# alexncoleman/WeaklySupervisedDL

Hardware: AMD Instinct MI355X
Metric: SegmentationModel train img/s at B=16 256x256 (higher is better)
Workload: dtype f32

## Files before the change

### include/wsdl_hip.h

```cpp
#ifndef WSDL_HIP_H
#define WSDL_HIP_H

#include <stddef.h>
#include <stdint.h>

#ifdef __cplusplus
extern "C" {
#endif

typedef void* wsdl_stream_t;

enum {
    WSDL_OK = 0,
    WSDL_EINVAL = -1,
    WSDL_EHIP = -2,
    WSDL_EWORKSPACE = -3
};

const char* wsdl_last_error(void);
int wsdl_launch_trace(int on);
const char* wsdl_last_launches(void);
int wsdl_version(void);
const char* wsdl_target_arch(void);

int wsdl_set_option(const char* name, int value);

enum { WSDL_PROF_IGEMM_128x128_A = 0,
       WSDL_PROF_IGEMM_128x128_U = 1,
       WSDL_PROF_IGEMM_128x64_A = 2, WSDL_PROF_IGEMM_128x64_U = 3,
       WSDL_PROF_IGEMM_64x256_A = 4, WSDL_PROF_IGEMM_64x256_U = 5,
       WSDL_PROF_IGEMM_64x128_A = 6, WSDL_PROF_IGEMM_64x128_U = 7,
       WSDL_PROF_WGRAD_128x128 = 8,
       WSDL_PROF_WGRAD_64x128 = 9,
       WSDL_PROF_WGRAD_FAST_128x128 = 10,
       WSDL_PROF_PAIRWISE = 11, WSDL_PROF_LAYERCAM = 12,
       WSDL_PROF_SPLIT_128x128 = 13,
       WSDL_PROF_SPLIT_128x64 = 14, WSDL_PROF_SPLIT_64x256 = 15, WSDL_PROF_SPLIT_64x128 = 16,
       WSDL_PROF_WGRAD_SPLIT32 = 17,
       WSDL_PROF_SPLIT_256x128 = 18,
       WSDL_PROF_STEM = 19,
       WSDL_PROF_WGRAD_SPLIT16D = 20,
       WSDL_PROF_SPLIT_GROUP = 21,
       WSDL_PROF_SPLIT_MULTI = 22,
       WSDL_PROF_NCLASSES = 23 };
const char* wsdl_prof_class_name(int cls);
int wsdl_prof_enable(int on);
int wsdl_prof_collect(int cls, long long* launches, double* total_ms, double* total_work,
                      double* total_work_executed ,
                      double* total_bytes );
int wsdl_prof_reset(void);

int wsdl_range_enable(int on);
int wsdl_range_push(const char* name);
int wsdl_range_pop(void);


size_t wsdl_conv2d_weight_layout_bytes(int Cout, int Cin, int kh, int kw, int dgrad, int* is_plain);
int wsdl_conv2d_prep_weights(const float* w, void* wt_fwd, void* wt_dgrad,
                             int Cout, int Cin, int kh, int kw,
                             const float* w_amax ,
                             wsdl_stream_t stream);

int wsdl_conv2d_fwd(const float* x, const void* wt_fwd, float* y,
                    int B, int Cin, int H, int W, int Cout, int kh, int kw,
                    int stride, int pad, int dil,
                    const float* scale, const float* shift, const float* residual, int relu,
                    long long x_bs, long long y_bs, long long res_bs,
                    const float* x_amax ,
                    float* y_amax ,
                    void* ws, size_t ws_bytes, wsdl_stream_t stream);
typedef struct wsdl_prep_desc {
    const float* w;
    void* wt_fwd;
    void* wt_dgrad;
    const float* w_amax;
    int Cout, Cin, taps, grid_x;
    int block_begin, reserved;
} wsdl_prep_desc;
int wsdl_conv2d_prep_weights_multi(const wsdl_prep_desc* desc, int n, int total_blocks, wsdl_stream_t stream);

size_t wsdl_conv2d_igemm_workspace(int B, int Cin, int H, int W, int Cout, int kh, int kw,
                                   int stride, int pad, int dil, int dgrad);

int wsdl_conv2d_dgrad(const float* dy, const void* wt_dgrad, float* dx,
                      int B, int Cin, int H, int W, int Cout, int kh, int kw,
                      int stride, int pad, int dil, int accumulate, const uint8_t* acc_mask,
                      long long dy_bs, const float* dy_amax, void* ws, size_t ws_bytes, wsdl_stream_t stream);
int wsdl_conv2d_fwd_group_ok(int n, int B, int Cin, int H, int W, int Cout);
size_t wsdl_conv2d_fwd_group_workspace(int n, const int* k, const int* dil, int B, int Cin, int H, int W, int Cout);
int wsdl_conv2d_fwd_group(int n, const float* x, const void* const* wt_fwd, float* const* y, const int* k, const int* dil,
                          int B, int Cin, int H, int W, int Cout, long long x_bs, const long long* y_bs,
                          const float* x_amax, void* ws, size_t ws_bytes, wsdl_stream_t stream);
int wsdl_conv2d_dgrad_multi_ok(int n, int B, int Cin, int H, int W, int Cout);
int wsdl_conv2d_dgrad_multi(int n, const float* const* dy, const void* const* wt_dgrad, const float* const* dy_amax,
                            const int* k, const int* dil, const long long* dy_bs, float* dx, int B, int Cin, int H, int W,
                            int Cout, int accumulate, wsdl_stream_t stream);

size_t wsdl_conv2d_wgrad_workspace(int B, int Cin, int H, int W, int Cout, int kh, int kw,
                                   int stride, int pad, int dil);
int wsdl_conv2d_wgrad(const float* x, const float* dy, float* dw,
                      int B, int Cin, int H, int W, int Cout, int kh, int kw,
                      int stride, int pad, int dil, int accumulate,
                      long long x_bs, long long dy_bs, const float* x_amax, const float* dy_amax,
                      void* ws, size_t ws_bytes, wsdl_stream_t stream);
size_t wsdl_conv2d_wgrad_presplit_bytes(int B, int Cin, int H, int W, int Cout, int kh, int kw, int stride, int pad, int dil);
int wsdl_conv2d_wgrad_ex(const float* x, const float* dy, float* dw, int B, int Cin, int H, int W,
                         int Cout, int kh, int kw, int stride, int pad, int dil, int accumulate,
                         long long x_bs, long long dy_bs, const float* x_amax, const float* dy_amax,
                         const float* x_chan_amax, const float* dy_chan_amax, const void* dy_presplit, void* ws,
                         size_t ws_bytes, wsdl_stream_t stream);

int wsdl_amax(const float* x, int B, long long per_image, long long x_bs, float* out, int zero_first,
              wsdl_stream_t stream);
int wsdl_multi_amax(const float* const* ptrs, const long long* counts, int n, float* out, wsdl_stream_t stream);

int wsdl_bias_grad(const float* dy, float* dbias, int B, int C, int HW, long long dy_bs,
                   int accumulate, wsdl_stream_t stream);

size_t wsdl_bn_workspace(int C);
int wsdl_bn_train_fwd(const float* x, const float* gamma, const float* beta, float* y,
                      float* save_mean, float* save_invstd, float* running_mean, float* running_var,
                      float momentum, float eps, int B, int C, int HW,
                      const float* residual, int relu, long long y_bs,
                      float* y_amax ,
                      uint8_t* relu_mask ,
                      void* ws, size_t ws_bytes,
                      float* chan_amax ,
// ... 365 lines not shown
```

### weaklysuperviseddl_amd/csrc/common.hip

```cpp
#include "common.h"

#include <dlfcn.h>

#include <algorithm>
#include <mutex>
#include <vector>

namespace wsdl {

static thread_local char g_err[512] = "";
Opt g_range_sentinel{0};

void set_error(const char* fmt, ...) {
    va_list ap;
    va_start(ap, fmt);
    vsnprintf(g_err, sizeof(g_err), fmt, ap);
    va_end(ap);
}

std::atomic<int> g_trace_launches{0};
static thread_local char g_trace[2048] = "";
static thread_local size_t g_trace_len = 0;
void trace_launch(const char* fmt, ...) {
    if (g_trace_len + 4 >= sizeof(g_trace)) return;
// ... 17 lines not shown
bool prof_enabled() { return g_prof_on; }

static bool g_ranges_on = false;
static int (*g_roctx_push)(const char*) = nullptr;
static int (*g_roctx_pop)() = nullptr;
static bool load_roctx() {
    if (g_roctx_push && g_roctx_pop) return true;
    for (const char* name : {"librocprofiler-sdk-roctx.so", "librocprofiler-sdk-roctx.so.1", "libroctx64.so", "libroctx64.so.4"}) {
        if (void* h = dlopen(name, RTLD_NOW | RTLD_GLOBAL)) {
            g_roctx_push = reinterpret_cast<int (*)(const char*)>(dlsym(h, "roctxRangePushA"));
            g_roctx_pop = reinterpret_cast<int (*)()>(dlsym(h, "roctxRangePop"));
            if (g_roctx_push && g_roctx_pop) return true;
        }
    }
    return false;
}

ProfScope::ProfScope(int c, hipStream_t st, double work, double work_executed, double bytes)
    : cls(c), s(st), slot(nullptr) {
    if (g_ranges_on) g_roctx_push(wsdl_prof_class_name(c));
    if (!g_prof_on) return;
    std::lock_guard<std::mutex> lk(g_prof_mu);
    ProfRec r;
    r.work = work;
    r.executed = work_executed >= 0.0 ? work_executed : work;
    r.bytes = bytes;
    if (!g_free_events.empty()) {
        r.start = g_free_events.back().first;
        r.stop = g_free_events.back().second;
        g_free_events.pop_back();
    } else {
        if (hipEventCreate(&r.start) != hipSuccess) return;
        if (hipEventCreate(&r.stop) != hipSuccess) return;
    }
    (void)hipEventRecord(r.start, s);
    g_prof[cls].push_back(r);
    slot = reinterpret_cast<void*>(g_prof[cls].size());
}

ProfScope::~ProfScope() {
    if (g_ranges_on) g_roctx_pop();
    if (!slot) return;
    std::lock_guard<std::mutex> lk(g_prof_mu);
    size_t idx = reinterpret_cast<size_t>(slot) - 1;
    if (idx < g_prof[cls].size()) (void)hipEventRecord(g_prof[cls][idx].stop, s);
}

}

extern "C" {

int wsdl_launch_trace(int on) {
    wsdl::g_trace_launches.store(on ? 1 : 0);
    wsdl::g_trace[0] = 0;
    wsdl::g_trace_len = 0;
    return WSDL_OK;
}

const char* wsdl_last_launches(void) {
    static thread_local char out[sizeof(wsdl::g_trace)];
    memcpy(out, wsdl::g_trace, sizeof(out));
    wsdl::g_trace[0] = 0;
    wsdl::g_trace_len = 0;
    return out;
}

const char* wsdl_last_error(void) { return wsdl::g_err; }
int wsdl_version(void) { return 201; }
const char* wsdl_target_arch(void) { return "gfx950"; }

const char* wsdl_prof_class_name(int cls) {
    static const char* names[WSDL_PROF_NCLASSES] = {
        "conv_igemm_fast_kernel<128, 128, 2, 16>", "conv_igemm_kernel<128, 128, 2, false>",
        "conv_igemm_fast_kernel<128, 64, 2, 32>", "conv_igemm_kernel<128, 64, 2, false>",
        "conv_igemm_fast_kernel<64, 256, 1, 16>", "conv_igemm_kernel<64, 256, 1, false>",
        "conv_igemm_fast_kernel<64, 128, 1, 32>", "conv_igemm_kernel<64, 128, 1, false>",
        "conv_wgrad_kernel<128, 128, 2>", "conv_wgrad_kernel<64, 128, 1>", "conv_wgrad_fast_kernel<128, 128, 2, 16>",
        "pairwise_kernel", "layercam_partial_kernel",
        "conv_igemm_split_kernel<128, 128, 2, 16, 256, AR>", "conv_igemm_split_kernel<128, 64, 2, 32, 256, AR>",
        "conv_igemm_split_kernel<64, 256, 1, 16, 256, AR>", "conv_igemm_split_kernel<64, 128, 1, 32, 256, AR>",
        "conv_wgrad_split16_kernel<128, 128, false>", "conv_igemm_split_kernel<256, 128, 4, BK, 512, AR, false, false>",
        "stem_conv7x7s2_kernel", "conv_wgrad_split16d_kernel<MODE, DYRAW>",
        "conv_igemm_split_group_kernel<256, 128, 4, 16, 512, AR, false>",
        "conv_igemm_split_kernel<256, 128, 4, 16, 512, AR, false, true>"};
    return cls >= 0 && cls < WSDL_PROF_NCLASSES ? names[cls] : "?";
}

int wsdl_range_enable(int on) {
    if (on && !wsdl::load_roctx()) {
        wsdl::set_error("range_enable: librocprofiler-sdk-roctx.so / libroctx64.so could not be loaded");
        return WSDL_EINVAL;
    }
    wsdl::g_ranges_on = on != 0;
    return WSDL_OK;
}
int wsdl_range_push(const char* name) {
    if (wsdl::g_ranges_on && name) wsdl::g_roctx_push(name);
    return WSDL_OK;
}
int wsdl_range_pop(void) {
    if (wsdl::g_ranges_on) wsdl::g_roctx_pop();
    return WSDL_OK;
}

int wsdl_prof_enable(int on) {
    std::lock_guard<std::mutex> lk(wsdl::g_prof_mu);
    wsdl::g_prof_on = on != 0;
    return WSDL_OK;
}

int wsdl_prof_reset(void) {
    std::lock_guard<std::mutex> lk(wsdl::g_prof_mu);
    for (auto& v : wsdl::g_prof) {
        for (auto& r : v) wsdl::g_free_events.emplace_back(r.start, r.stop);
        v.clear();
    }
    return WSDL_OK;
}

int wsdl_prof_collect(int cls, long long* launches, double* total_ms, double* total_work,
                      double* total_work_executed, double* total_bytes) {
    WSDL_REQUIRE(cls >= 0 && cls < WSDL_PROF_NCLASSES, "prof class %d out of range", cls);
    std::lock_guard<std::mutex> lk(wsdl::g_prof_mu);
    double ms = 0.0, work = 0.0, exe = 0.0, byt = 0.0;
    for (auto& r : wsdl::g_prof[cls]) {
        WSDL_HIP_CHECK(hipEventSynchronize(r.stop));
        float t = 0.f;
        WSDL_HIP_CHECK(hipEventElapsedTime(&t, r.start, r.stop));
        ms += t;
        work += r.work;
        exe += r.executed;
        byt += r.bytes;
    }
    if (launches) *launches = (long long)wsdl::g_prof[cls].size();
    if (total_ms) *total_ms = ms;
    if (total_work) *total_work = work;
    if (total_work_executed) *total_work_executed = exe;
    if (total_bytes) *total_bytes = byt;
    return WSDL_OK;
}

}
```

### weaklysuperviseddl_amd/csrc/conv_igemm.hip

```cpp
#include "common.h"

#include <type_traits>
#include <algorithm>
#include <cstdint>
#include <mutex>

typedef float f32x16 __attribute__((ext_vector_type(16)));

namespace {

constexpr int kThreads = 256;

struct ConvSrc {
    const float* x;
    const float* wt;
    const float* x_amax;
    int KH, KW, bh, ch, K, Cin;
    long long x_bs;
    unsigned x_bytes;
};

struct ConvP {
    const float* x;
    const float* wt;
// ... 492 lines not shown
    const int OHOW = p.OH * p.OW;
    float vmax = 0.f;
    for (long long idx = blockIdx.x * (long long)blockDim.x + threadIdx.x; idx < total;
         idx += (long long)gridDim.x * blockDim.x) {
        const int co = (int)(idx / p.P), pix = (int)(idx - (long long)co * p.P);
        float v = 0.f;
        for (int z = 0; z < p.ksplit; ++z) v += p.slab[(long long)z * total + idx];
        const int ob = pix / OHOW, orp = pix - ob * OHOW;
        if (p.scale) v *= p.scale[co];
        if (p.shift) v += p.shift[co];
        const long long off = (long long)co * OHOW + orp;
        if (p.res) v += p.res[(long long)ob * p.res_bs + off];
        float* y = p.y + (long long)ob * p.y_bs + off;
        if (p.accumulate) v += acc_prev(p, y);
        if (p.relu) v = fmaxf(v, 0.f);
        *y = v;
        vmax = fmaxf(vmax, fabsf(v));
    }
    if (p.y_amax) publish_amax(vmax, p.y_amax);
}

__global__ void conv_splitk_reduce_vec4_kernel(ConvP p) {
    const int OHOW = p.OH * p.OW;
    float vmax = 0.f;
    const long long total = (long long)p.Cout * p.P, total4 = total / 4;
    const float4* slab4 = reinterpret_cast<const float4*>(p.slab);
    for (long long i4 = blockIdx.x * (long long)blockDim.x + threadIdx.x; i4 < total4;
         i4 += (long long)gridDim.x * blockDim.x) {
        const long long idx = i4 * 4;
        const int co = (int)(idx / p.P), pix = (int)(idx - (long long)co * p.P);
        float4 v = slab4[i4];
        for (int z = 1; z < p.ksplit; ++z) {
            const float4 t = slab4[(long long)z * total4 + i4];
            v.x += t.x; v.y += t.y; v.z += t.z; v.w += t.w;
        }
        const int ob = pix / OHOW, orp = pix - ob * OHOW;
        if (p.scale) { const float sc = p.scale[co]; v.x *= sc; v.y *= sc; v.z *= sc; v.w *= sc; }
        if (p.shift) { const float sh = p.shift[co]; v.x += sh; v.y += sh; v.z += sh; v.w += sh; }
        const long long off = (long long)co * OHOW + orp;
        if (p.res) {
            const float4 r = *reinterpret_cast<const float4*>(p.res + (long long)ob * p.res_bs + off);
            v.x += r.x; v.y += r.y; v.z += r.z; v.w += r.w;
        }
        float4* y = reinterpret_cast<float4*>(p.y + (long long)ob * p.y_bs + off);
        if (p.accumulate) {
            float4 o = *y;
            if (p.acc_mask) {
                const long long e = reinterpret_cast<const float*>(y) - p.acc_base;
                const unsigned nb = ((unsigned)p.acc_mask[e >> 3] >> (unsigned)(e & 4)) & 0xFu;
                if (!(nb & 1u)) o.x = 0.f;
                if (!(nb & 2u)) o.y = 0.f;
                if (!(nb & 4u)) o.z = 0.f;
                if (!(nb & 8u)) o.w = 0.f;
            }
            v.x += o.x; v.y += o.y; v.z += o.z; v.w += o.w;
        }
        if (p.relu) { v.x = fmaxf(v.x, 0.f); v.y = fmaxf(v.y, 0.f); v.z = fmaxf(v.z, 0.f); v.w = fmaxf(v.w, 0.f); }
        *y = v;
        vmax = amax4(vmax, v);
    }
    if (p.y_amax) publish_amax(vmax, p.y_amax);
}

struct WgradP {
    const float* x;
    const float* dy;
    float* slab;
    int B, Cin, H, W, Cout, OH, OW, KH, KW, stride, pad, dil;
    int N;
    int P;
    int chunks_per_split;
    long long x_bs, dy_bs;
    unsigned x_bytes, dy_bytes;
    int ow0, own;
    int slab0;
    int xcd_order;
    int nb, splits;
    int b_ow0[4], b_own[4], b_cps[4];
    const float* x_amax;
    int xa_stride, da_stride;
};

#include "conv_split.h"

template <int BM, int BN, int WM>
__global__ __launch_bounds__(kThreads) void conv_wgrad_kernel(WgradP p) {
    constexpr int BK = 32, LD = BK + 1;
    constexpr int WN = 4 / WM, MI = BM / WM / 32, NI = BN / WN / 32;
    constexpr int A_PER = BM / 8, B_PER = BN / 8;
    static_assert(MI >= 1 && NI >= 1 && MI * 32 * WM == BM && NI * 32 * WN == BN, "bad tile");

    extern __shared__ __attribute__((aligned(16))) float wg_lds[];
    float* const As0 = wg_lds;
    float* const Bs0 = wg_lds + 2 * BM * LD;

    const int tid = threadIdx.x;
    const int lane = tid & 63, wid = tid >> 6;
    const int wm = wid / WN, wn = wid % WN;
    const int n0 = blockIdx.x * BN, m0 = blockIdx.y * BM;
    const int OHOW = p.OH * p.OW, HW = p.H * p.W;
    const int px = tid & 31, row0 = tid >> 5;

    int b_shift[B_PER];
    int b_coff[B_PER];
#pragma unroll
    for (int e = 0; e < B_PER; ++e) {
        const int n = n0 + row0 + 8 * e;
        if (n < p.N) {
            const int tap = n / p.Cin, ci = n - tap * p.Cin;
            const int ti = tap / p.KW, tj = tap - ti * p.KW;
            const int dh = ti * p.dil - p.pad, dw = tj * p.dil - p.pad;
            b_shift[e] = (int)(((unsigned)dh << 16) | ((unsigned)dw & 0xffffu));
            b_coff[e] = ci * HW;
        } else {
            b_shift[e] = 0;
            b_coff[e] = -1;
        }
    }
    const int n_last = min(n0 + BN, p.N) - 1;
    const int tap0 = n0 / p.Cin;
    const bool single_tap = tap0 == n_last / p.Cin;
    const int t_dh = (tap0 / p.KW) * p.dil - p.pad, t_dw = (tap0 % p.KW) * p.dil - p.pad;

    f32x16 acc[MI][NI];
#pragma unroll
    for (int i = 0; i < MI; ++i)
#pragma unroll
        for (int j = 0; j < NI; ++j)
#pragma unroll
            for (int r = 0; r < 16; ++r) acc[i][j][r] = 0.f;

    float ra[A_PER], rb[B_PER];
    const int chunk_begin = blockIdx.z * p.chunks_per_split;
    const int total_chunks = (p.P + BK - 1) / BK;
    const int chunk_end = min(chunk_begin + p.chunks_per_split, total_chunks);

    auto next_valid = [&](int c) {
        if (!single_tap) return min(c, chunk_end);
        for (; c < chunk_end; ++c) {
            const int pix = c * BK + px;
            bool ok = pix < p.P;
            if (ok) {
                const int pb = pix / OHOW, rp = pix - pb * OHOW;
                const int oh = rp / p.OW, ow = rp - oh * p.OW;
                const int ih = oh * p.stride + t_dh, iw = ow * p.stride + t_dw;
                ok = ih >= 0 && ih < p.H && iw >= 0 && iw < p.W;
            }
            if (__any(ok)) break;
        }
        return c;
    };

    auto load_tiles = [&](int chunk) {
        const int pix = chunk * BK + px;
        const bool ok = pix < p.P;
        int pb = 0, oh = 0, ow = 0, rp = 0;
        if (ok) {
            pb = pix / OHOW;
            rp = pix - pb * OHOW;
            oh = rp / p.OW;
            ow = rp - oh * p.OW;
        }
        const float* dyb = p.dy + (long long)pb * p.dy_bs + rp;
#pragma unroll
        for (int e = 0; e < A_PER; ++e) {
            const int co = m0 + row0 + 8 * e;
// ... 582 lines not shown
    else if (g_conv_arith)
        hipLaunchKernelGGL((conv_igemm_split_kernel<BM, BN, WM, BK, kThreads, 1, MF>), grid, dim3(kThreads), 0, s, p);
    else
        hipLaunchKernelGGL((conv_igemm_split_kernel<BM, BN, WM, BK, kThreads, 0>), grid, dim3(kThreads), 0, s, p);
    WSDL_LAUNCH_CHECK();
    return WSDL_OK;
}

wsdl::Opt g_conv_il{1};
int launch_split_256x128(const ConvP& p_in, hipStream_t s) {
    ConvP p = p_in;
    dim3 grid(p.grid_x > 0 ? p.grid_x : wsdl::cdiv(p.P, 128), wsdl::cdiv(p.Cout, 256), p.ksplit > 1 ? p.ksplit : 1);
    p.xcd_py = choose_xcd_py(p, grid.x, grid.y);
    p.xcd_rowfast = 0;
    p.tile_img_major = 0;
    if (p.nsrc > 0 && grid.y % 2 == 0 && ((long long)grid.x * grid.y) % 8 == 0) {
        int py = 4;
        while (py > 1 && (grid.y % py || grid.x % (8 / py))) py /= 2;
        if (grid.y % py == 0 && grid.x % (8 / py) == 0) {
            p.xcd_py = py;
            p.xcd_rowfast = 1;
        }
    }
    WSDL_TRACE("split<256,128,16> ar=%d il=%d nsrc=%d ks=%d xcd_py=%d rowfast=%d imgmajor=%d nb=%d grid=%ux%ux%u", (int)g_conv_arith,
               (int)(g_conv_arith == 1 && g_conv_il), p.nsrc, p.ksplit, p.xcd_py, p.xcd_rowfast, p.tile_img_major, p.nb, grid.x, grid.y, grid.z);
    if (p.nsrc > 0) {
        if (g_conv_arith == 2) hipLaunchKernelGGL((conv_igemm_split_kernel<256, 128, 4, 16, 512, 2, false, true>), grid, dim3(512), 0, s, p);
        else if (g_conv_arith && g_conv_il)
            hipLaunchKernelGGL((conv_igemm_split_kernel<256, 128, 4, 16, 512, 1, false, true, true>), grid, dim3(512), 0, s, p);
        else if (g_conv_arith) hipLaunchKernelGGL((conv_igemm_split_kernel<256, 128, 4, 16, 512, 1, false, true>), grid, dim3(512), 0, s, p);
        else hipLaunchKernelGGL((conv_igemm_split_kernel<256, 128, 4, 16, 512, 0, false, true>), grid, dim3(512), 0, s, p);
        WSDL_LAUNCH_CHECK();
        return WSDL_OK;
    }
    if (g_conv_arith == 2) hipLaunchKernelGGL((conv_igemm_split_kernel<256, 128, 4, 16, 512, 2>), grid, dim3(512), 0, s, p);
    else if (g_conv_arith && g_conv_il)
        hipLaunchKernelGGL((conv_igemm_split_kernel<256, 128, 4, 16, 512, 1, false, false, true>), grid, dim3(512), 0, s, p);
    else if (g_conv_arith) hipLaunchKernelGGL((conv_igemm_split_kernel<256, 128, 4, 16, 512, 1>), grid, dim3(512), 0, s, p);
    else hipLaunchKernelGGL((conv_igemm_split_kernel<256, 128, 4, 16, 512, 0>), grid, dim3(512), 0, s, p);
    WSDL_LAUNCH_CHECK();
    return WSDL_OK;
}

template <int BM, int BN, int WM>
int launch_cfg(const ConvP& p, hipStream_t s, bool aligned, bool split) {
    dim3 grid(p.grid_x > 0 ? p.grid_x : wsdl::cdiv(p.P, BN), wsdl::cdiv(p.Cout, BM));
    constexpr bool kSmallTile = BM * BN <= 128 * 64;
    if (split) {
        if constexpr (kSmallTile) {
            if (p.Cin % 32 == 0) {
                return launch_split<BM, BN, WM, 32>(p, s, grid);
            }
        }
        return launch_split<BM, BN, WM, 16>(p, s, grid);
    } else if (aligned) {
        if constexpr (kSmallTile) {
            if (p.Cin % 32 == 0) {
                return launch_fast<BM, BN, WM, 32>(p, s, grid);
            }
        }
        return launch_fast<BM, BN, WM, 16>(p, s, grid);
    } else {
        WSDL_TRACE("fp32_generic<%d,%d> grid=%ux%u", BM, BN, grid.x, grid.y);
        hipLaunchKernelGGL((conv_igemm_kernel<BM, BN, WM, false>), grid, dim3(kThreads), 0, s, p);
    }
    WSDL_LAUNCH_CHECK();
    return WSDL_OK;
}

wsdl::Opt g_ksplit_target{512}, g_ksplit_max{8}, g_ksplit_min_chunks{4};
int igemm_ksplit(int P, int Cout, int Cin, int T, int dil) {
    if (Cin % 32 != 0 || Cout % 4 != 0 || Cout <= 64) return 1;
    const long long blocks = (long long)wsdl::cdiv(P, 64) * wsdl::cdiv(Cout, 128);
    const int nq = T * (Cin / 32);
    const long long b128 = (long long)wsdl::cdiv(P, 128) * wsdl::cdiv(Cout, 128);
    if (b128 >= 200 && b128 < g_tile_threshold && nq >= 64) return 2;
    if (blocks >= 160 || nq < 8) return 1;
    long long s = g_ksplit_target / blocks;
    if (s > nq / g_ksplit_min_chunks) s = nq / g_ksplit_min_chunks;
    if (s > g_ksplit_max) s = g_ksplit_max;
    return s < 2 ? 1 : (int)s;
}

int launch_igemm(const ConvP& p_in, hipStream_t s, double flops, void* ws, size_t ws_bytes) {
    ConvP p = p_in;
    p.ksplit = 1;
    p.slab = nullptr;
    p.ow0 = 0;
    p.own = p.OW;
    p.nb = 1;
    p.grid_x = 0;
    p.xcd_py = 0;
    {
        const int ks = igemm_ksplit(p.P, p.Cout, p.Cin, p.KH * p.KW, p.bh < 0 ? -p.bh : p.bh);
        if (ks > 1 && ws && ws_bytes >= (size_t)ks * p.Cout * p.P * sizeof(float) && p.x_bytes != 0 &&
            (long long)p.K * p.Cout * 4 < (1ll << 31)) {
            p.ksplit = ks;
            p.slab = static_cast<float*>(ws);
        }
    }
    const bool split = split_eligible(p.Cout, p.Cin, p.KH * p.KW);
    if (split && p.x_bytes == 0) {
        wsdl::set_error("conv: activation extent >= 2 GiB is not supported by the split-bf16 kernels "
                        "(wsdl_set_option(\"conv_split\", 0) selects the fp32 kernels)");
        return WSDL_EINVAL;
    }
    if (split && g_conv_arith && !p.x_amax) {
        wsdl::set_error("conv: the fp16x2 split kernels need the activation tensor's amax (x_amax / dy_amax is null)");
        return WSDL_EINVAL;
    }
    float* amax_after = nullptr;
    if (p.y_amax && !(split && p.ksplit == 1) && p.ksplit == 1) {
        amax_after = p.y_amax;
        p.y_amax = nullptr;
    }
    const bool aligned = split || ((p.Cin % 16) == 0 && (p.Cout % 4) == 0 && p.x_bytes != 0 &&
                                   (long long)p.K * p.Cout * 4 < (1ll << 31));
    const long long kWant = g_tile_threshold;
    int cfg;
    if (p.Cout <= 64)
        cfg = (long long)wsdl::cdiv(p.P, 256) * wsdl::cdiv(p.Cout, 64) >= kWant ? 2 : 3;
    else
        cfg = ((long long)wsdl::cdiv(p.P, 128) * wsdl::cdiv(p.Cout, 128) * p.ksplit >= kWant) ? 0 : 1;
    Band bands[8];
    int nb = 1;
    bands[0] = Band{0, p.OW};
    if (aligned) nb = column_bands(p.OW, p.W, p.ah, p.bh, p.ch, p.sh, p.KW, bands);
    const bool t256 = cfg == 0 && split && p.Cout * 10 >= wsdl::cdiv(p.Cout, 256) * 256 * 9 &&
                      (long long)wsdl::cdiv(p.P, 128) * wsdl::cdiv(p.Cout, 256) * p.ksplit >= 256;
    if (cfg == 1 && split && g_conv_arith >= 1 && p.Cin % 32 == 0 && p.Cout % 64 == 0 && p.ksplit == 1 &&
        p.nsrc == 0 && (long long)wsdl::cdiv(p.P, 64) * wsdl::cdiv(p.Cout, 128) < kWant)
        cfg = 4;
    const int bn_tile = cfg == 0 ? 128 : (cfg == 1 || cfg == 4) ? 64 : cfg == 2 ? 256 : 128;
    double executed = flops;
    if (aligned && wsdl::prof_enabled()) {
        executed = 0.0;
        for (int i = 0; i < nb; ++i) {
            ConvP q = p;
            q.ow0 = bands[i].ow0; q.own = bands[i].own; q.P = p.B * p.OH * q.own;
            executed += flops * ((double)q.own / p.OW) * igemm_executed_fraction(q, bn_tile);
        }
    }
    const double bytes = 4.0 * ((double)p.B * p.Cin * p.H * p.W + (double)p.K * p.Cout + (double)p.P * p.Cout * (p.res ? 2 : 1));
    wsdl::ProfScope prof(t256 ? (p.nsrc > 0 ? WSDL_PROF_SPLIT_MULTI : WSDL_PROF_SPLIT_256x128)
                              : split ? WSDL_PROF_SPLIT_128x128 + (cfg == 4 ? 1 : cfg) : WSDL_PROF_IGEMM_128x128_A + cfg * 2 + (aligned ? 0 : 1),
                         s, flops, executed, bytes);
    {
        ConvP q = p;
        q.nb = nb;
        int tiles = 0;
        for (int i = 0; i < nb && nb > 1; ++i) {
            q.b_ow0[i] = bands[i].ow0;
            q.b_own[i] = bands[i].own;
            q.b_tile0[i] = tiles;
            tiles += wsdl::cdiv((long long)p.B * p.OH * bands[i].own, bn_tile);
        }
        q.b_tile0[nb > 1 ? nb : 0] = tiles;
        q.grid_x = nb > 1 ? tiles : 0;
        int rc;
        if (p.nsrc > 0 && !t256) {
            wsdl::set_error("conv: a multi-source launch needs the 256x128 split form (rows a multiple of 256, >= 256 tiles)");
            return WSDL_EINVAL;
        }
        if (t256) {
            rc = launch_split_256x128(q, s);
        } else
        switch (cfg) {
            case 0: rc = launch_cfg<128, 128, 2>(q, s, aligned, split); break;
            case 1: rc = launch_cfg<128, 64, 2>(q, s, aligned, split); break;
            case 2: rc = launch_cfg<64, 256, 1>(q, s, aligned, split); break;
            case 4: rc = launch_split<64, 64, 2, 32>(q, s, dim3(q.grid_x > 0 ? q.grid_x : wsdl::cdiv(q.P, 64), wsdl::cdiv(q.Cout, 64))); break;
            default: rc = launch_cfg<64, 128, 1>(q, s, aligned, split); break;
        }
        if (rc) return rc;
    }
    if (p.ksplit > 1) {
        const long long total = (long long)p.Cout * p.P;
        const bool vec4 = (p.OH * p.OW) % 4 == 0 && p.y_bs % 4 == 0 && (!p.res || p.res_bs % 4 == 0) &&
                          (reinterpret_cast<uintptr_t>(p.y) & 15) == 0 && (!p.res || (reinterpret_cast<uintptr_t>(p.res) & 15) == 0);
        WSDL_TRACE("splitk_reduce%s", vec4 ? "_vec4" : "");
        if (vec4)
            hipLaunchKernelGGL(conv_splitk_reduce_vec4_kernel, dim3((int)std::min<long long>((total / 4 + 255) / 256, 8192)),
                               dim3(256), 0, s, p);
        else
            hipLaunchKernelGGL(conv_splitk_reduce_kernel, dim3((int)std::min<long long>((total + 255) / 256, 4096)),
                               dim3(256), 0, s, p);
    }
    WSDL_LAUNCH_CHECK();
    if (amax_after) {
        const long long per = (long long)p.Cout * p.OH * p.OW, total = (long long)p.B * per;
        hipLaunchKernelGGL(amax_kernel, dim3((int)std::min<long long>((total + 1023) / 1024, 2048)), dim3(256), 0, s, p.y, per,
                           p.y_bs, total, amax_after);
        WSDL_LAUNCH_CHECK();
// ... 202 lines not shown
__global__ void transpose_add_kernel(const float* __restrict__ t, float* __restrict__ dw, int Cout, int Cin,
                                     int accumulate) {
    __shared__ float tile[32][33];
    const int co0 = blockIdx.x * 32, ci0 = blockIdx.y * 32;
    for (int r = threadIdx.y; r < 32; r += 8) {
        const int ci = ci0 + r, co = co0 + threadIdx.x;
        tile[r][threadIdx.x] = (ci < Cin && co < Cout) ? t[(long long)ci * Cout + co] : 0.f;
    }
    __syncthreads();
    for (int r = threadIdx.y; r < 32; r += 8) {
        const int co = co0 + r, ci = ci0 + threadIdx.x;
        if (co < Cout && ci < Cin) {
            const long long o = (long long)co * Cin + ci;
            dw[o] = accumulate ? dw[o] + tile[threadIdx.x][r] : tile[threadIdx.x][r];
        }
    }
}

bool wgrad_role_swap(int Cin, int Cout, int kh, int kw, int stride, int pad) {
    return kh == 1 && kw == 1 && stride == 1 && pad == 0 && !wgrad_chunk32(Cout, Cin, Cin) && wgrad_chunk32(Cin, Cout, Cout);
}

enum { WGRAD_REDUCE_PLAIN = 0, WGRAD_REDUCE_TILED, WGRAD_REDUCE_VEC4, WGRAD_REDUCE_MANY, WGRAD_REDUCE_MANY16 };
struct WgradReduce {
    const float* slab;
    float* dw;
    unsigned long long live;
    int S, Cout, Cin, T;
    int accumulate, kind;
    int grid_x, nblocks;
};
int wgrad_reduce_one(const WgradReduce& d, hipStream_t s) {
    switch (d.kind) {
        case WGRAD_REDUCE_TILED:
            hipLaunchKernelGGL(wgrad_reduce_tiled_kernel, dim3(d.grid_x, d.Cout), dim3(256), 0, s, d.slab, d.dw, d.S, d.Cout, d.Cin, d.T,
                               d.accumulate, d.live);
            break;
        case WGRAD_REDUCE_VEC4:
            hipLaunchKernelGGL(wgrad_reduce_vec4_kernel, dim3(d.nblocks), dim3(256), 0, s, reinterpret_cast<const float4*>(d.slab),
                               reinterpret_cast<float4*>(d.dw), d.S, (long long)d.Cout * d.Cin * d.T / 4, d.accumulate);
            break;
        case WGRAD_REDUCE_MANY:
            hipLaunchKernelGGL(wgrad_reduce_many_kernel, dim3(d.nblocks), dim3(256), 0, s, d.slab, d.dw, d.S, d.Cout, d.Cin, d.T,
                               d.accumulate, d.live);
            break;
        case WGRAD_REDUCE_MANY16:
            hipLaunchKernelGGL(wgrad_reduce_many16_kernel, dim3(d.nblocks), dim3(256), 0, s, d.slab, d.dw, d.S, d.Cout, d.Cin, d.T,
                               d.accumulate, d.live);
            break;
        default:
            hipLaunchKernelGGL(wgrad_reduce_kernel, dim3(d.nblocks), dim3(256), 0, s, d.slab, d.dw, d.S, d.Cout, d.Cin, d.T, d.accumulate,
                               d.live);
            break;
    }
    WSDL_LAUNCH_CHECK();
    return WSDL_OK;
}

template <int BM, int BN, int WM>
int launch_wgrad_fast(const WgradP& p, hipStream_t s, int S) {
    dim3 grid(p.N / BN, p.Cout / BM, S);
    hipLaunchKernelGGL((conv_wgrad_fast_kernel<BM, BN, WM, 16>), grid, dim3(kThreads), 2 * (BM + BN) * 17 * sizeof(float), s, p);
    WSDL_LAUNCH_CHECK();
    return WSDL_OK;
}

}

extern "C" {

int wsdl_set_option(const char* name, int value) {
    WSDL_REQUIRE(name, "set_option: null name");
    static std::mutex mu;
    std::lock_guard<std::mutex> lock(mu);
    WSDL_REQUIRE(wsdl::g_plans_recording.load() == 0,
                 "set_option(%s): a launch plan is being recorded (its launches are chosen under ONE option set)", name);
    if (!strcmp(name, "tile_threshold")) { g_tile_threshold = value; return WSDL_OK; }
    if (!strcmp(name, "conv_split")) { g_conv_split = value != 0; return WSDL_OK; }
    if (!strcmp(name, "stem_kernel")) { g_stem_kernel = value != 0; return WSDL_OK; }
    if (!strcmp(name, "wgrad_direct")) { g_wgrad_direct = value; return WSDL_OK; }
    if (!strcmp(name, "wgrad_chan_scale")) { g_wgrad_chan_scale = value != 0; return WSDL_OK; }
    if (!strcmp(name, "wgrad_dyraw")) { g_wgrad_dyraw = value; return WSDL_OK; }
    if (!strcmp(name, "conv_il")) { g_conv_il = value != 0; return WSDL_OK; }
    if (!strcmp(name, "xcd_map")) { g_xcd_map = value; return WSDL_OK; }
    if (!strcmp(name, "ksplit_target")) { g_ksplit_target = value; return WSDL_OK; }
    if (!strcmp(name, "ksplit_max")) { g_ksplit_max = value; return WSDL_OK; }
    if (!strcmp(name, "ksplit_min_chunks")) { g_ksplit_min_chunks = value > 0 ? value : 1; return WSDL_OK; }
    if (!strcmp(name, "conv_arith")) {
        WSDL_REQUIRE(value >= 0 && value <= 2, "conv_arith: 0 (bf16x3), 1 (fp16x2), 2 (fp16x2, low piece at 2^11)");
        g_conv_arith = value;
        return WSDL_OK;
    }
    if (!strcmp(name, "range_sentinel")) { wsdl::g_range_sentinel = value != 0; return WSDL_OK; }
    if (!strcmp(name, "group_tps10")) { g_group_tps10 = value > 0 ? value : 45; return WSDL_OK; }
    if (!strcmp(name, "bn_resident")) { wsdl::g_bn_resident = value; return WSDL_OK; }
    if (!strcmp(name, "bn_wide_c")) { wsdl::g_bn_wide_c = value; return WSDL_OK; }
    if (!strcmp(name, "layercam_tail_mod")) {
        WSDL_REQUIRE(value >= 0 && value <= 32, "layercam_tail_mod: 0..32");
        wsdl::g_layercam_tail_mod = value;
        return WSDL_OK;
    }
    if (!strcmp(name, "wgrad_split")) { g_wgrad_split = value != 0; return WSDL_OK; }
    if (!strcmp(name, "wgrad_xcd")) { g_wgrad_xcd = value; return WSDL_OK; }
    if (!strcmp(name, "wgrad_min_tiles")) { g_wgrad_min_tiles = value > 0 ? value : 1; return WSDL_OK; }
    if (!strcmp(name, "wgrad_blocks")) { g_wgrad_blocks = value > 0 ? value : 768; return WSDL_OK; }
    wsdl::set_error("set_option: unknown option %s", name);
    return WSDL_EINVAL;
}

size_t wsdl_conv2d_weight_layout_bytes(int Cout, int Cin, int kh, int kw, int dgrad, int* is_plain) {
    const int T = kh * kw;
    const bool split = dgrad ? split_eligible(Cin, Cout, T) : split_eligible(Cout, Cin, T);
    if (is_plain) *is_plain = split ? 0 : 1;
    const size_t n = (size_t)Cout * Cin * T;
    return split ? (size_t)split_layout_bytes(g_conv_arith, (long long)T * (dgrad ? Cout : Cin), dgrad ? Cin : Cout) : n * 4;
}

int wsdl_conv2d_prep_weights(const float* w, void* wt_fwd, void* wt_dgrad, int Cout, int Cin,
                             int kh, int kw, const float* w_amax, wsdl_stream_t stream) {
    WSDL_REQUIRE(w && (wt_fwd || wt_dgrad), "prep_weights: null pointer");
    WSDL_REQUIRE(Cout > 0 && Cin > 0 && kh > 0 && kw > 0, "prep_weights: bad shape");
    const long long total = (long long)Cout * Cin * kh * kw;
    const int T = kh * kw;
    const bool fwd_split = wt_fwd && split_eligible(Cout, Cin, T);
    const bool dg_split = wt_dgrad && split_eligible(Cin, Cout, T);
    float* pf = fwd_split ? nullptr : static_cast<float*>(wt_fwd);
    float* pd = dg_split ? nullptr : static_cast<float*>(wt_dgrad);
    if (fwd_split || dg_split) {
        dim3 grid(wsdl::cdiv(Cin, 32), wsdl::cdiv(Cout, 32));
        unsigned char* f8 = fwd_split ? static_cast<unsigned char*>(wt_fwd) : nullptr;
        unsigned char* d8 = dg_split ? static_cast<unsigned char*>(wt_dgrad) : nullptr;
        if (g_conv_arith) {
            const float* amax = w_amax;
            if (!amax) {
                const long long body = f8 ? split_layout_bytes(1, (long long)T * Cin, Cout) - 16
                                          : split_layout_bytes(1, (long long)T * Cout, Cin) - 16;
                float* tr = reinterpret_cast<float*>((f8 ? f8 : d8) + body);
                WSDL_HIP_CHECK(hipMemsetAsync(tr, 0, 16, wsdl::as_stream(stream)));
                hipLaunchKernelGGL(amax_kernel, dim3((int)std::min<long long>((total + 1023) / 1024, 1024)), dim3(256), 0,
                                   wsdl::as_stream(stream), w, total, total, total, tr);
                amax = tr;
            }
            if (g_conv_arith == 2)
                hipLaunchKernelGGL(prep_weights_split_kernel<2>, grid, dim3(256), 0, wsdl::as_stream(stream), w, f8, d8, Cout, Cin,
                                   T, amax);
            else
                hipLaunchKernelGGL(prep_weights_split_kernel<1>, grid, dim3(256), 0, wsdl::as_stream(stream), w, f8, d8, Cout, Cin,
                                   T, amax);
        } else {
            hipLaunchKernelGGL(prep_weights_split_kernel<0>, grid, dim3(256), 0, wsdl::as_stream(stream), w, f8, d8, Cout, Cin,
                               T, static_cast<const float*>(nullptr));
        }
        WSDL_LAUNCH_CHECK();
    }
    if (pf || pd) {
        if (T <= 9 && Cout <= 65535 * 32) {
            dim3 grid(wsdl::cdiv(Cin, 32), wsdl::cdiv(Cout, 32));
            if (T == 1)
                hipLaunchKernelGGL((prep_weights_tiled_kernel<1>), grid, dim3(32, 8), 0, wsdl::as_stream(stream), w, pf,
                                   pd, Cout, Cin, T);
            else
                hipLaunchKernelGGL((prep_weights_tiled_kernel<9>), grid, dim3(32, 8), 0, wsdl::as_stream(stream), w, pf,
                                   pd, Cout, Cin, T);
        } else {
            const int blocks = (int)std::min<long long>((total + 255) / 256, 4096);
            hipLaunchKernelGGL(prep_weights_kernel, dim3(blocks), dim3(256), 0, wsdl::as_stream(stream), w, pf, pd,
// ... 795 lines not shown
```

### weaklysuperviseddl_amd/csrc/conv_split.h

```cpp
#pragma once

typedef __bf16 bf16x8 __attribute__((ext_vector_type(8)));
typedef __bf16 bf16x2 __attribute__((ext_vector_type(2)));
typedef _Float16 half8 __attribute__((ext_vector_type(8)));
typedef float f32x4 __attribute__((ext_vector_type(4)));

__device__ __forceinline__ void split3(float x0, float x1, unsigned& h, unsigned& m, unsigned& l) {
    f32x2 v = {x0, x1};
    h = __builtin_bit_cast(unsigned, __builtin_convertvector(v, bf16x2));
    f32x2 r = {x0 - __builtin_bit_cast(float, h << 16), x1 - __builtin_bit_cast(float, h & 0xffff0000u)};
    m = __builtin_bit_cast(unsigned, __builtin_convertvector(r, bf16x2));
    f32x2 s = {r[0] - __builtin_bit_cast(float, m << 16), r[1] - __builtin_bit_cast(float, m & 0xffff0000u)};
    l = __builtin_bit_cast(unsigned, __builtin_convertvector(s, bf16x2));
}

__device__ __forceinline__ void split2hs(float x0, float x1, unsigned& h, unsigned& l) {
    f32x2 v = {x0, x1};
    const half2v hv = __builtin_convertvector(v, half2v);
    h = __builtin_bit_cast(unsigned, hv);
    f32x2 r = {(x0 - (float)hv[0]) * 2048.f, (x1 - (float)hv[1]) * 2048.f};
    l = __builtin_bit_cast(unsigned, __builtin_convertvector(r, half2v));
}

template <int AR> struct SplitArith;
template <> struct SplitArith<0> {
    static constexpr int NP = 3;
    using frag = bf16x8;
    static __device__ __forceinline__ f32x16 mma(frag a, frag b, f32x16 c) {
        return __builtin_amdgcn_mfma_f32_32x32x16_bf16(a, b, c, 0, 0, 0);
    }
};
template <> struct SplitArith<1> {
    static constexpr int NP = 2;
    using frag = half8;
    static __device__ __forceinline__ f32x16 mma(frag a, frag b, f32x16 c) {
        return __builtin_amdgcn_mfma_f32_32x32x16_f16(a, b, c, 0, 0, 0);
    }
};
template <> struct SplitArith<2> : SplitArith<1> {};
template <int AR, typename F>
__device__ __forceinline__ f32x16 split_products(const F (&a)[SplitArith<AR>::NP], const F (&b)[SplitArith<AR>::NP], f32x16 c) {
    using A = SplitArith<AR>;
    if constexpr (AR == 0) {
        c = A::mma(a[2], b[0], c);
        c = A::mma(a[0], b[2], c);
        c = A::mma(a[1], b[1], c);
        c = A::mma(a[1], b[0], c);
        c = A::mma(a[0], b[1], c);
        c = A::mma(a[0], b[0], c);
    } else {
        c = A::mma(a[1], b[0], c);
        c = A::mma(a[0], b[1], c);
        c = A::mma(a[0], b[0], c);
    }
    return c;
}

constexpr int split_k16_bytes(int AR) { return AR ? 64 : 96; }
__host__ __device__ constexpr long long split_layout_bytes(int AR, long long k_total, long long rows) {
    return (k_total / 16) * rows * split_k16_bytes(AR) + 16;
}

template <int BM, int BN, int WM, int BK, int NT, int AR, bool MF, bool MS, bool IL>
__device__ __forceinline__ void conv_igemm_split_body(const ConvP& p, const int bx_in, const int by_in, const int bz,
                                                      const int grid_x, const int grid_y) {
    static_assert(!MF || (AR >= 1 && BK == 32), "16x16x32 form: fp16x2, K chunk 32");
    using Ar = SplitArith<AR>;
    using frag = typename Ar::frag;
    constexpr int NP = Ar::NP;
    constexpr int K16B = split_k16_bytes(AR);
    constexpr int WN = (NT / 64) / WM;
    constexpr int MI = BM / WM / 32, NI = BN / WN / 32;
    static_assert(MI >= 1 && NI >= 1 && MI * 32 * WM == BM && NI * 32 * WN == BN, "bad tile");
    static_assert(BK == 16 || BK == 32, "K chunk");
    constexpr int KS = BK / 16;
    constexpr int ROW = MF ? 128 : KS * K16B + 16;
    constexpr int UPR = K16B / 16;
    constexpr int A_UPS = BM * UPR;
    constexpr int A_U = (KS * A_UPS + NT - 1) / NT;
    constexpr bool A_EXACT = A_U * NT == KS * A_UPS;
    constexpr int B_STEP = NT / BN;
    constexpr int B_PER = BK / B_STEP;
    static_assert(B_PER == 4 || B_PER == 8 || B_PER == 16 || B_PER == 32, "B tile");
    constexpr unsigned kOOB = 0x80000000u;

    __shared__ __attribute__((aligned(16))) unsigned char As[2][BM * ROW];
    __shared__ __attribute__((aligned(16))) unsigned char Bs[2][BN * ROW];
    __shared__ int vtaps[64];

    const int tid = threadIdx.x;
    const int lane = tid & 63, wid = tid >> 6;
    const int wm = wid / WN, wn = wid % WN;
    int bx = bx_in, by = by_in;
    if (p.xcd_py > 0) {
        const int gx = grid_x;
        const int L = by * gx + bx;
        const int xcd = L & 7, idx = L >> 3;
        const int py = p.xcd_py, px = 8 / py;
        const int lx = gx / px, ly = grid_y / py;
        if (p.xcd_rowfast) {
            bx = (xcd / py) * lx + idx / ly;
            by = (xcd % py) * ly + idx % ly;
        } else {
            bx = (xcd / py) * lx + idx % lx;
            by = (xcd % py) * ly + idx / lx;
        }
    }
    const int m0 = by * BM;
    int w_ow0 = p.ow0, w_own = p.own, w_tile0 = 0;
    if (p.nb > 1) {
        w_ow0 = p.b_ow0[0];
        w_own = p.b_own[0];
#pragma unroll
        for (int i = 1; i < 4; ++i)
            if (i < p.nb && bx >= p.b_tile0[i]) {
                w_ow0 = p.b_ow0[i];
                w_own = p.b_own[i];
                w_tile0 = p.b_tile0[i];
            }
    }
    const int W_P = p.nb > 1 ? p.B * p.OH * w_own : p.P;
    int lt = bx - w_tile0;
    if (p.tile_img_major) {
        const int ohw = p.OH * w_own;
        const int tpi = ohw / BN;
        if (tpi > 1 && tpi * BN == ohw) lt = (lt % p.B) * tpi + lt / p.B;
    }
    const int n0 = lt * BN;
    const int OHOW = p.OH * p.OW;
    const int HW = p.H * p.W;

    const int pl = tid % BN;
    const int kr = tid / BN;
    const int pix = n0 + pl;
    const bool pix_ok = pix < W_P;
    int pb = 0, poh = 0, pow_ = 0;
    const int OHW = p.OH * w_own;
    if (pix_ok) {
        pb = pix / OHW;
        const int r = pix - pb * OHW;
        poh = r / w_own;
        pow_ = w_ow0 + (r - poh * w_own);
    }
// ... 1290 lines not shown
```

### weaklysuperviseddl_amd/ops.py

```python
import ctypes as C

import os

import threading

import numpy as np
import torch

from ._lib import lib, check, WsdlError

_vp = C.c_void_p


_raw_stream = torch._C._cuda_getCurrentRawStream
_cur_device = torch._C._cuda_getDevice


def raw_stream(device=None):
    idx = device.index if (device is not None and device.index is not None) else _cur_device()
    return _raw_stream(idx)


def _stream():
    return _raw_stream(_cur_device())
# ... 4353 lines not shown
class _Fanout(torch.autograd.Function):

    @staticmethod
    def forward(ctx, x, n):
        ctx.set_materialize_grads(False)
        outs = tuple(_alias(x) for _ in range(n))
        a = getattr(x, "_wsdl_amax", None)
        if a is not None and getattr(x, "_wsdl_amax_version", x._version) == x._version:
            for o in outs:
                _publish_amax(o, a)
        return outs

    @staticmethod
    def backward(ctx, *gs):
        gs = [_dense(g, "gradient") for g in gs if g is not None]
        if not gs:
            return None, None
        if len(gs) == 1:
            return gs[0], None
        acc = torch.empty_like(gs[0])
        check(lib().wsdl_add(_p(gs[0]), _p(gs[1]), _p(acc), acc.numel(), 0, _stream()))
        for g in gs[2:]:
            check(lib().wsdl_add(_p(acc), _p(g), _p(acc), acc.numel(), 0, _stream()))
        return acc, None


def fanout(x, n=2):
    if not (torch.is_grad_enabled() and x.requires_grad and x.is_cuda):
        return (x,) * n
    return _Fanout.apply(x, int(n))


def add_scalars(a, b):
    return _AddAct.apply(a.reshape(1), b.reshape(1), False).reshape(())


def kl_div_batchmean(xn, s):
    return _KLDivBatchMean.apply(xn, s)


RANGES = [False]


def ranges_enable(on=True):
    check(lib().wsdl_range_enable(int(bool(on))))
    RANGES[0] = bool(on)


class prof_range:
    __slots__ = ("name",)

    def __init__(self, name):
        self.name = name

    def __enter__(self):
        if RANGES[0]:
            lib().wsdl_range_push(self.name.encode())

    def __exit__(self, *exc):
        if RANGES[0]:
            lib().wsdl_range_pop()
        return False


if os.environ.get("WSDL_ROCTX") == "1":
    try:
        ranges_enable(True)
    except Exception:
        RANGES[0] = False


PROF_ON = [False]


def prof_enable(on):
    check(lib().wsdl_prof_enable(int(on)))
    PROF_ON[0] = bool(on)


def prof_reset():
    check(lib().wsdl_prof_reset())


PROF_NCLASSES = 23


def prof_class_name(cls):
    return lib().wsdl_prof_class_name(int(cls)).decode()


def prof_collect(cls):
    n, ms, work, exe, byt = C.c_longlong(0), C.c_double(0), C.c_double(0), C.c_double(0), C.c_double(0)
    check(lib().wsdl_prof_collect(int(cls), C.byref(n), C.byref(ms), C.byref(work), C.byref(exe), C.byref(byt)))
    return n.value, ms.value, work.value, exe.value, byt.value
```

Before: 906.0.

## Add direct 3x3 stride-1 conv kernel staging split-fp16 input halo tiles in LDS

Adds a specialized kernel for 3x3, stride-1, same-size convolutions with small channel counts (Cin<=128, Cout<=128) on the fp16x2 split path. It loads a spatial input tile with a one-pixel halo once into LDS, already converted to hi/lo fp16 pairs. All nine filter taps then read shifted fragments from that tile, instead of gathering im2col rows from global memory for every tap. Weight fragments are prefetched three deep, and the same fused epilogue (scale, shift, residual, relu, amax) is applied. It is on by default, and it risks lower occupancy because of the large LDS footprint and launch_bounds(...,1), plus extra edge-case handling for borders.

Result: no change. 908.8 (median of 6 runs) (+0.3%).

```diff
diff --git a/include/wsdl_hip.h b/include/wsdl_hip.h
--- a/include/wsdl_hip.h
+++ b/include/wsdl_hip.h
@@ -42,7 +42,8 @@
        WSDL_PROF_WGRAD_SPLIT16D = 20,
        WSDL_PROF_SPLIT_GROUP = 21,
        WSDL_PROF_SPLIT_MULTI = 22,
-       WSDL_PROF_NCLASSES = 23 };
+       WSDL_PROF_RES3X3 = 23,
+       WSDL_PROF_NCLASSES = 24 };
 const char* wsdl_prof_class_name(int cls);
 int wsdl_prof_enable(int on);
 int wsdl_prof_collect(int cls, long long* launches, double* total_ms, double* total_work,
diff --git a/weaklysuperviseddl_amd/csrc/common.hip b/weaklysuperviseddl_amd/csrc/common.hip
--- a/weaklysuperviseddl_amd/csrc/common.hip
+++ b/weaklysuperviseddl_amd/csrc/common.hip
@@ -123,7 +123,7 @@
         "conv_wgrad_split16_kernel<128, 128, false>", "conv_igemm_split_kernel<256, 128, 4, BK, 512, AR, false, false>",
         "stem_conv7x7s2_kernel", "conv_wgrad_split16d_kernel<MODE, DYRAW>",
         "conv_igemm_split_group_kernel<256, 128, 4, 16, 512, AR, false>",
-        "conv_igemm_split_kernel<256, 128, 4, 16, 512, AR, false, true>"};
+        "conv_igemm_split_kernel<256, 128, 4, 16, 512, AR, false, true>", "conv_res3x3_kernel<WM> (fp16x2 split)"};
     return cls >= 0 && cls < WSDL_PROF_NCLASSES ? names[cls] : "?";
 }
 
diff --git a/weaklysuperviseddl_amd/csrc/conv_igemm.hip b/weaklysuperviseddl_amd/csrc/conv_igemm.hip
--- a/weaklysuperviseddl_amd/csrc/conv_igemm.hip
+++ b/weaklysuperviseddl_amd/csrc/conv_igemm.hip
@@ -598,6 +598,7 @@
 };
 
 #include "conv_split.h"
+#include "conv_res3x3.h"
 
 template <int BM, int BN, int WM>
 __global__ __launch_bounds__(kThreads) void conv_wgrad_kernel(WgradP p) {
@@ -1346,6 +1347,42 @@
     return s < 2 ? 1 : (int)s;
 }
 
+wsdl::Opt g_conv_res3x3{1};
+bool res3x3_eligible(const ConvP& p, bool split) {
+    return g_conv_res3x3 && split && g_conv_arith == 1 && p.KH == 3 && p.KW == 3 && p.sh == 1 && p.ah == 1 &&
+           (p.bh == 1 || p.bh == -1) && p.ch == -p.bh &&
+           p.OH == p.H && p.OW == p.W && p.Cin % 32 == 0 && p.Cin <= 128 && p.Cout % 64 == 0 && p.Cout <= 128 &&
+           p.ksplit == 1 && p.nsrc == 0 && p.x_bytes != 0;
+}
+
+int launch_res3x3(const ConvP& p, hipStream_t s, double flops) {
+    const bool tall = p.Cin <= 64;
+    const int tr = tall ? 8 : 4;
+    const int tiles_w = wsdl::cdiv(p.OW, kRes3TC), tiles_h = wsdl::cdiv(p.OH, tr);
+    const long long blocks = (long long)p.B * tiles_h * tiles_w * (p.Cout / 64);
+    WSDL_REQUIRE(blocks < (1ll << 31), "conv: too many 3x3 tiles");
+    const int lds = res3x3_lds_bytes(p.Cin, tr);
+    static std::once_flag once;
+    static hipError_t attr_rc = hipSuccess;
+    std::call_once(once, [] {
+        attr_rc = hipFuncSetAttribute(reinterpret_cast<const void*>(&conv_res3x3_kernel<1>), hipFuncAttributeMaxDynamicSharedMemorySize,
+                                      res3x3_lds_bytes(64, 8));
+        if (attr_rc == hipSuccess)
+            attr_rc = hipFuncSetAttribute(reinterpret_cast<const void*>(&conv_res3x3_kernel<2>),
+                                          hipFuncAttributeMaxDynamicSharedMemorySize, res3x3_lds_bytes(128, 4));
+    });
+    WSDL_HIP_CHECK(attr_rc);
+    const double bytes = 4.0 * ((double)p.B * p.Cin * p.H * p.W + (double)p.K * p.Cout + (double)p.P * p.Cout * (p.res ? 2 : 1));
+    wsdl::ProfScope prof(WSDL_PROF_RES3X3, s, flops, flops, bytes);
+    WSDL_TRACE("split<64,%dx%d,32> res3x3 ar=1 mfma16x16x32 cin=%d lds=%d grid=%u", tr, kRes3TC, p.Cin, lds, (unsigned)blocks);
+    if (tall)
+        hipLaunchKernelGGL(conv_res3x3_kernel<1>, dim3((unsigned)blocks), dim3(kThreads), lds, s, p, tiles_w, tiles_h);
+    else
+        hipLaunchKernelGGL(conv_res3x3_kernel<2>, dim3((unsigned)blocks), dim3(kThreads), lds, s, p, tiles_w, tiles_h);
+    WSDL_LAUNCH_CHECK();
+    return WSDL_OK;
+}
+
 int launch_igemm(const ConvP& p_in, hipStream_t s, double flops, void* ws, size_t ws_bytes) {
     ConvP p = p_in;
     p.ksplit = 1;
@@ -1373,6 +1410,7 @@
         wsdl::set_error("conv: the fp16x2 split kernels need the activation tensor's amax (x_amax / dy_amax is null)");
         return WSDL_EINVAL;
     }
+    if (res3x3_eligible(p, split)) return launch_res3x3(p, s, flops);
     float* amax_after = nullptr;
     if (p.y_amax && !(split && p.ksplit == 1) && p.ksplit == 1) {
         amax_after = p.y_amax;
@@ -1741,6 +1779,7 @@
     if (!strcmp(name, "wgrad_chan_scale")) { g_wgrad_chan_scale = value != 0; return WSDL_OK; }
     if (!strcmp(name, "wgrad_dyraw")) { g_wgrad_dyraw = value; return WSDL_OK; }
     if (!strcmp(name, "conv_il")) { g_conv_il = value != 0; return WSDL_OK; }
+    if (!strcmp(name, "conv_res3x3")) { g_conv_res3x3 = value != 0; return WSDL_OK; }
     if (!strcmp(name, "xcd_map")) { g_xcd_map = value; return WSDL_OK; }
     if (!strcmp(name, "ksplit_target")) { g_ksplit_target = value; return WSDL_OK; }
     if (!strcmp(name, "ksplit_max")) { g_ksplit_max = value; return WSDL_OK; }
diff --git a/weaklysuperviseddl_amd/csrc/conv_res3x3.h b/weaklysuperviseddl_amd/csrc/conv_res3x3.h
--- /dev/null
+++ b/weaklysuperviseddl_amd/csrc/conv_res3x3.h
@@ -0,0 +1,162 @@
+#pragma once
+
+constexpr int kRes3TC = 32;
+constexpr int kRes3HC = kRes3TC + 2;
+constexpr int res3x3_row_units(int cin) { return cin / 4 + 1; }
+constexpr int res3x3_lds_bytes(int cin, int tr) { return (tr + 2) * kRes3HC * res3x3_row_units(cin) * 16; }
+
+template <int WM>
+__global__ __launch_bounds__(kThreads, 1) void conv_res3x3_kernel(ConvP p, int tiles_w, int tiles_h) {
+    constexpr int WN = 4 / WM, TR = 2 * WN, HR = TR + 2;
+    constexpr int TMI = 64 / WM / 16, TNI = 4;
+    constexpr unsigned kOOB = 0x80000000u;
+    extern __shared__ __attribute__((aligned(16))) unsigned char res3_lds[];
+    u32x4* const lds_st = reinterpret_cast<u32x4*>(res3_lds);
+    const half8* const lds_rd = reinterpret_cast<const half8*>(res3_lds);
+
+    const int tid = threadIdx.x;
+    const int lane = tid & 63, wid = tid >> 6;
+    const int wm = wid / WN, wn = wid % WN;
+    const int l15 = lane & 15, lh = lane >> 4;
+    const int ny = p.Cout / 64;
+    int L = blockIdx.x;
+    const int m0 = (L % ny) * 64;
+    L /= ny;
+    const int tw = L % tiles_w;
+    L /= tiles_w;
+    const int th = L % tiles_h, b = L / tiles_h;
+    const int oh0 = th * TR, ow0 = tw * kRes3TC;
+    const int Cin = p.Cin, HW = p.H * p.W, OHOW = p.OH * p.OW;
+    const int RU = res3x3_row_units(Cin);
+
+    const int wbytes = (p.K / 16) * p.Cout * 64;
+    const __amdgpu_buffer_rsrc_t rx = __builtin_amdgcn_make_buffer_rsrc(const_cast<float*>(p.x), 0, (int)p.x_bytes, 0x00020000);
+    const __amdgpu_buffer_rsrc_t rw = __builtin_amdgcn_make_buffer_rsrc(const_cast<float*>(p.wt), 0, wbytes, 0x00020000);
+    int ex, ew;
+    const float xs = pow2_scale(*p.x_amax, ex);
+    (void)pow2_scale(*reinterpret_cast<const float*>(reinterpret_cast<const unsigned char*>(p.wt) + wbytes), ew);
+    const float out_scale = pow2(-(ex + ew));
+
+    {
+        const bool vec = (p.W & 3) == 0 && (p.x_bs & 3) == 0 && (reinterpret_cast<uintptr_t>(p.x) & 15) == 0;
+        const int items = (Cin / 8) * HR * 10;
+        const long long img = (long long)b * p.x_bs;
+        for (int it = tid; it < items; it += kThreads) {
+            const int g = it % 10, rest = it / 10;
+            const int hr = rest % HR, cg = rest / HR;
+            const int hc0 = g == 0 ? 0 : g == 9 ? kRes3HC - 1 : 1 + 4 * (g - 1);
+            const int nc = (g == 0 || g == 9) ? 1 : 4;
+            const int ih = oh0 - 1 + hr, iw0 = ow0 - 1 + hc0;
+            const bool row_ok = ih >= 0 && ih < p.H;
+            const long long base = img + (long long)cg * 8 * HW + (long long)ih * p.W + iw0;
+            float v[8][4];
+            if (nc == 4 && vec) {
+                const unsigned voff = (row_ok && iw0 < p.W) ? (unsigned)base * 4u : kOOB;
+#pragma unroll
+                for (int e = 0; e < 8; ++e) {
+                    const f32x4 q = __builtin_bit_cast(f32x4, __builtin_amdgcn_raw_buffer_load_b128(rx, voff, (unsigned)(e * HW) * 4u, 0));
+#pragma unroll
+                    for (int c = 0; c < 4; ++c) v[e][c] = q[c];
+                }
+            } else {
+#pragma unroll
+                for (int c = 0; c < 4; ++c) {
+                    if (c < nc) {
+                        const bool ok = row_ok && iw0 + c >= 0 && iw0 + c < p.W;
+                        const unsigned voff = ok ? (unsigned)(base + c) * 4u : kOOB;
+#pragma unroll
+                        for (int e = 0; e < 8; ++e)
+                            v[e][c] = __builtin_bit_cast(float, __builtin_amdgcn_raw_buffer_load_b32(rx, voff, (unsigned)(e * HW) * 4u, 0));
+                    }
+                }
+            }
+            const int unit = (hr * kRes3HC + hc0) * RU + (cg >> 2) * 8 + (cg & 3);
+#pragma unroll
+            for (int c = 0; c < 4; ++c) {
+                if (c < nc) {
+                    unsigned h[4], l[4];
+#pragma unroll
+                    for (int e = 0; e < 4; ++e) split2h(v[2 * e][c] * xs, v[2 * e + 1][c] * xs, h[e], l[e]);
+                    lds_st[unit + c * RU] = u32x4{h[0], h[1], h[2], h[3]};
+                    lds_st[unit + c * RU + 4] = u32x4{l[0], l[1], l[2], l[3]};
+                }
+            }
+        }
+    }
+    __syncthreads();
+
+    f32x4 acc[TMI][TNI];
+#pragma unroll
+    for (int i = 0; i < TMI; ++i)
+#pragma unroll
+        for (int j = 0; j < TNI; ++j)
+#pragma unroll
+            for (int r = 0; r < 4; ++r) acc[i][j][r] = 0.f;
+
+    const unsigned voff_a = (unsigned)((m0 + wm * (64 / WM) + l15) * 64 + (lh & 1) * 16 + (lh >> 1) * p.Cout * 64);
+    int unit_b[TNI];
+#pragma unroll
+    for (int j = 0; j < TNI; ++j) unit_b[j] = ((2 * wn + (j >> 1) + 1) * kRes3HC + 16 * (j & 1) + l15 + 1) * RU + lh;
+
+    struct Frags {
+        half8 a[TMI][2], x[TNI][2];
+    };
+    const int cpt = Cin / 32, nq = 9 * cpt;
+    auto load_frags = [&](Frags& f, int q) {
+        const int t = q / cpt, c = q - t * cpt;
+        const int ti = t / 3, tj = t - ti * 3;
+        const int dy = ti * p.bh + p.ch, dx = tj * p.bh + p.ch;
+        const unsigned soff = (unsigned)(((t * Cin + c * 32) >> 4) * p.Cout * 64);
+#pragma unroll
+        for (int i = 0; i < TMI; ++i)
+#pragma unroll
+            for (int pc = 0; pc < 2; ++pc)
+                f.a[i][pc] = __builtin_bit_cast(half8, __builtin_amdgcn_raw_buffer_load_b128(rw, voff_a + (unsigned)(i * 16 * 64 + pc * 32), soff, 0));
+        const int shift = (dy * kRes3HC + dx) * RU + c * 8;
+#pragma unroll
+        for (int j = 0; j < TNI; ++j)
+#pragma unroll
+            for (int pc = 0; pc < 2; ++pc) f.x[j][pc] = lds_rd[unit_b[j] + shift + pc * 4];
+    };
+    auto mfma_step = [&](const Frags& f) {
+#pragma unroll
+        for (int i = 0; i < TMI; ++i)
+#pragma unroll
+            for (int j = 0; j < TNI; ++j) {
+                f32x4 c = acc[i][j];
+                c = __builtin_amdgcn_mfma_f32_16x16x32_f16(f.a[i][1], f.x[j][0], c, 0, 0, 0);
+                c = __builtin_amdgcn_mfma_f32_16x16x32_f16(f.a[i][0], f.x[j][1], c, 0, 0, 0);
+                c = __builtin_amdgcn_mfma_f32_16x16x32_f16(f.a[i][0], f.x[j][0], c, 0, 0, 0);
+                acc[i][j] = c;
+            }
+    };
+    Frags f0, f1, f2;
+    load_frags(f0, 0);
+    __builtin_amdgcn_sched_barrier(0);
+    load_frags(f1, 1);
+    __builtin_amdgcn_sched_barrier(0);
+    for (int q = 0; q < nq; q += 3) {
+        load_frags(f2, q + 2);
+        __builtin_amdgcn_sched_barrier(0);
+        mfma_step(f0);
+        __builtin_amdgcn_sched_barrier(0);
+        load_frags(f0, min(q + 3, nq - 1));
+        __builtin_amdgcn_sched_barrier(0);
+        mfma_step(f1);
+        __builtin_amdgcn_sched_barrier(0);
+        load_frags(f1, min(q + 4, nq - 1));
+        __builtin_amdgcn_sched_barrier(0);
+        mfma_step(f2);
+        __builtin_amdgcn_sched_barrier(0);
+    }
+
+    float vmax = 0.f;
+#pragma unroll
+    for (int j = 0; j < TNI; ++j) {
+        const int oh = oh0 + 2 * wn + (j >> 1), ow = ow0 + 16 * (j & 1) + l15;
+        if (oh >= p.OH || ow >= p.OW) continue;
+        split_store_pixel<1, TMI, 4, 16>(p, b, oh * p.OW + ow, OHOW, m0 + wm * (64 / WM), out_scale, [&](int r) { return lh * 4 + r; },
+                                         vmax, [&](int i, int r) { return acc[i][j][r]; });
+    }
+    if (p.y_amax) publish_amax(vmax, p.y_amax);
+}
diff --git a/weaklysuperviseddl_amd/csrc/conv_split.h b/weaklysuperviseddl_amd/csrc/conv_split.h
--- a/weaklysuperviseddl_amd/csrc/conv_split.h
+++ b/weaklysuperviseddl_amd/csrc/conv_split.h
@@ -59,6 +59,31 @@
 constexpr int split_k16_bytes(int AR) { return AR ? 64 : 96; }
 __host__ __device__ constexpr long long split_layout_bytes(int AR, long long k_total, long long rows) {
     return (k_total / 16) * rows * split_k16_bytes(AR) + 16;
+}
+
+template <int AR, int TMI, int RT, int TS, typename RowFn, typename ValFn>
+__device__ __forceinline__ void split_store_pixel(const ConvP& p, int ob, int orp, int OHOW, int co0, float out_scale, RowFn acc_row,
+                                                  float& vmax, ValFn value) {
+    float* yb = p.y + (long long)ob * p.y_bs + orp;
+    const float* rbp = p.res ? p.res + (long long)ob * p.res_bs + orp : nullptr;
+#pragma unroll
+    for (int i = 0; i < TMI; ++i) {
+#pragma unroll
+        for (int r = 0; r < RT; ++r) {
+            const int co = co0 + i * TS + acc_row(r);
+            if (co >= p.Cout) continue;
+            float v = value(i, r);
+            if constexpr (AR >= 1) v *= out_scale;
+            if (p.scale) v *= p.scale[co];
+            if (p.shift) v += p.shift[co];
+            const long long off = (long long)co * OHOW;
+            if (rbp) v += rbp[off];
+            if (p.accumulate) v += acc_prev(p, yb + off);
+            if (p.relu) v = fmaxf(v, 0.f);
+            yb[off] = v;
+            vmax = fmaxf(vmax, fabsf(v));
+        }
+    }
 }
 
 template <int BM, int BN, int WM, int BK, int NT, int AR, bool MF, bool MS, bool IL>
diff --git a/weaklysuperviseddl_amd/ops.py b/weaklysuperviseddl_amd/ops.py
--- a/weaklysuperviseddl_amd/ops.py
+++ b/weaklysuperviseddl_amd/ops.py
@@ -4459,7 +4459,7 @@
     check(lib().wsdl_prof_reset())
 
 
-PROF_NCLASSES = 23
+PROF_NCLASSES = 24
 
 
 def prof_class_name(cls):
```
